# Gyeeta/gyeeta

Hardware: AMD Instinct MI355X
Metric: events/sec ingested + p50/p99 quantile error vs reference, 1→8 MI355X (higher is better)
Workload: dtype int64; 1 GPU; C3/C4: 10000 hosts x 1000 services, raw 24-B tcp_ipv4_resp_event_t stream, uniform over services, 1 window (ingest + window close) per step; service_keys_total=10000000, multi_level_windows=0, td_pend_cap=1920, td_pend_cap_is_library_default=False, exchange=none, exchange_requested=none, exchange_fallback=False

## Files before the change

gyeeta_amd/csrc/gys_kernels.hpp:

```cpp
#pragma once

#include "gys_device.hpp"

namespace gys {

#define GYS_HUGE_VALUE_BITS 20
#define GYS_HUGE_BINS (1u << GYS_HUGE_VALUE_BITS)
#define GYS_ROW_BITS 6
#define GYS_ROW_MASK 0x3Fu
#define GYS_ROW_V6 0x20u
#define GYS_BM_WORDS 32u
#define GYS_STAGED_WORD(tresp, cli_port) ((uint64_t)(((uint32_t)(tresp) << GYS_ROW_BITS) | ((uint32_t)(cli_port) & 0x1Fu)))
#define GYS_STAGED_WORD_FAM(tresp, cli_port, v6) ((uint32_t)(((uint32_t)(tresp) << GYS_ROW_BITS) | ((v6) ? GYS_ROW_V6 : 0u) | ((uint32_t)(cli_port) & 0x1Fu)))

enum { CTR_RESP_EVENTS = 0, CTR_RESP_DROP_RANGE, CTR_RESP_DROP_NOLISTENER, CTR_CONN_EVENTS, CTR_CONN_UNKNOWN, CTR_LSTATE_RECORDS,
       CTR_LSTATE_MISSED, CTR_LSTATE_ERRORS, CTR_LSTATE_DELETED, CTR_TD_MERGES, CTR_TD_MERGE_VALUES, CTR_ACTCONN_RECORDS, CTR_ACTCONN_REMOTE_LISTEN, CTR_ACTCONN_UNKNOWN,
       CTR_CONN_NEW, CTR_CONN_CLOSED, CTR_CONN_CLOSED_NO_NOTIFY, CTR_CONN_CLI_SIDE, CTR_RESP_RUN_OVERFLOW, CTR_NUM };

__global__ void k_table_set(DevTable t, const uint64_t *kv, uint32_t n)
{
	const uint32_t i = blockIdx.x * blockDim.x + threadIdx.x;
	if (i >= n) return;
	const uint64_t key = kv[2u * i];
	uint32_t h = get_uint64_hash(key) & t.mask;
// ... 1219 lines not shown
			const bool fq_on = !SPILL && t0 + 2ull * TILE < e1;
			if (fq_on) {
#pragma unroll
				for (uint32_t j = 0; j < NQ; ++j) fq[j] = ((const uint4 *)p.hll32)[(tile_no & 3u) * ((1u << GYS_HLL_P) / 16u) + j * T + tid];
			}
			for (uint32_t eb0 = 0; eb0 < ntile; eb0 += (uint32_t)FU * T) {
				uint32_t kk[FU], vv[FU];
				uint64_t dd[FU];
#pragma unroll
				for (int j = 0; j < FU; ++j) {
					const uint32_t e = eb0 + (uint32_t)j * T + tid;
					const uint32_t ee = e < ntile ? e : TILE;
					kk[j] = s_key[ee];
					vv[j] = s_val[ee];
				}
				GYS_MEM_FENCE();
#pragma unroll
				for (int j = 0; j < FU; ++j) dd[j] = s_dst[kk[j]];
				GYS_MEM_FENCE();
#pragma unroll
				for (int j = 0; j < FU; ++j) {
					const uint32_t e = eb0 + (uint32_t)j * T + tid;
					if (e < ntile && dd[j]) dstb[dd[j] + e] = vv[j];
				}
			}
			if (fq_on) {
				uint32_t mn = 0xFFFFFFFFu;
#pragma unroll
				for (uint32_t j = 0; j < NQ; ++j) mn = min(min(mn, min(fq[j].x, fq[j].y)), min(fq[j].z, fq[j].w));
				mn = wave_min_u32(mn);
				if (lane == 0) {
					const uint32_t qn = tile_no & 3u;
					atomicMin(&s_fqm[qn], mn);
					atomicMin(&s_floor[tile_no & 1u], min(min(mn, s_fqm[(qn + 1u) & 3u]), min(s_fqm[(qn + 2u) & 3u], s_fqm[(qn + 3u) & 3u])));
				}
			}
		}
		GYS_TICK(11);
	}
#ifdef GYS_RESP_TIMING
	if (!SPILL && lane == 0) {
#pragma unroll
		for (int i = 0; i < 12; ++i) atomicAdd(&g_resp_timing[i], (unsigned long long)tacc[i]);
		atomicAdd(&g_resp_timing[15], 1ull);
	}
#endif
	if (SPILL) return;
	if (DBG && dbg_sink == 0xDEADBEEFu) p.counters[CTR_RESP_EVENTS] = 1;
	if (wmax >= 0) tmax = wmax >> GYS_ROW_BITS;
	tmax = wave_max_i32(tmax);
	if (lane == 0 && tmax != INT32_MIN) atomicMax(&s_gmax, tmax);
	if (ndrop_range) atomicAdd(&s_drop[0], ndrop_range);
	if (ndrop_nol) atomicAdd(&s_drop[1], ndrop_nol);
	__syncthreads();
	if (tid < 64u) {
		unsigned long long cnt = 0, sum = 0;
		if (tid < 15u) {
			for (uint32_t w = 0; w < 16u; ++w) {
				const unsigned long long v = s_gh[w * GYS_GH_STRIDE + tid];
				cnt += v >> 40;
				sum += v & ((1ull << 40) - 1);
			}
			if (cnt) {
				atomicAdd(&p.ghist[2 * tid], cnt);
				atomicAdd(&p.ghist[2 * tid + 1], sum);
			}
		}
		unsigned long long tot = cnt;
#pragma unroll
		for (int d = 8; d >= 1; d >>= 1) tot += (unsigned long long)__shfl_xor((long long)tot, d, 64);
		if (tid == 0 && tot) atomicAdd(&p.ghist[30], tot);
	}
	if (!SHARED) {
		constexpr int KMAX = (int)(2048u / T);
		bool fvalid[KMAX];
		uint32_t fkey[KMAX], fcur[KMAX];
#pragma unroll
		for (int j = 0; j < KMAX; ++j) {
			const uint32_t k = (uint32_t)j * T + tid;
			fvalid[j] = k < L;
			fkey[j] = fvalid[j] ? s_slot[k] : 0u;
			fcur[j] = fvalid[j] ? s_cur[k] : 0u;
		}
		finalize_keys_wg<true, KMAX>(p.fin, &s_fin, tid, lane, fvalid, fkey, fcur);
	}
	if (tid == 0) {
		if (s_gmax != INT32_MIN) atomicMax(p.gmax, (long long)s_gmax);
		if (hd.part == 0u) atomicAdd((unsigned long long *)&p.counters[CTR_RESP_EVENTS], (unsigned long long)(e1 - e0));
		if (s_drop[0]) atomicAdd((unsigned long long *)&p.counters[CTR_RESP_DROP_RANGE], (unsigned long long)s_drop[0]);
		if (s_drop[1]) atomicAdd((unsigned long long *)&p.counters[CTR_RESP_DROP_NOLISTENER], (unsigned long long)s_drop[1]);
	}
}

struct AppendP {
	uint32_t *batch_cnt;
	const uint32_t *off_end;
	const uint32_t *staged;
	uint32_t *td_cur;
	uint32_t *td_pend;
	uint32_t pcap, nsvc;
};

__global__ __launch_bounds__(256) void k_key_append(AppendP p)
{
	const uint32_t lane = threadIdx.x & 63u;
	const uint32_t nchunks = (p.nsvc + 63u) / 64u, nwaves = gridDim.x * 4u;
	for (uint32_t chunk = blockIdx.x * 4u + (threadIdx.x >> 6); chunk < nchunks; chunk += nwaves) {
		const uint32_t key = chunk * 64u + lane;
		const uint32_t m = key < p.nsvc ? p.batch_cnt[key] : 0u;
		unsigned long long todo = __ballot(m != 0);
		if (!todo) continue;
		const uint32_t oend = m ? p.off_end[key] : 0u;
		const uint32_t cur = m ? p.td_cur[key] : 0u;
		if (m) {
			p.batch_cnt[key] = 0;
			p.td_cur[key] = cur + m;
		}
		while (todo) {
			const int k = __ffsll((long long)todo) - 1;
			todo &= todo - 1;
			const uint32_t km = (uint32_t)__shfl((int)m, k, 64), ke = (uint32_t)__shfl((int)oend, k, 64), kc = (uint32_t)__shfl((int)cur, k, 64);
			if ((uint64_t)kc + km > (uint64_t)p.pcap) continue;
			const uint32_t *src = p.staged + (ke - km);
			uint32_t *dst = p.td_pend + (size_t)(chunk * 64u + (uint32_t)k) * p.pcap + kc;
			for (uint32_t i = lane; i < km; i += 64u) dst[i] = src[i];
		}
	}
}

struct DigestP {
	int64_t *td_sum;
	uint32_t *td_cnt;
	TdMeta *td_meta;
	int2 *td_minmax;
	uint32_t *td_pend;
	uint32_t *td_cur;
	uint32_t pcap, nsvc;
	uint32_t pend_cap;
	const uint32_t *staged;
	gys_hist_rec *hist_win, *hist_all;
	uint32_t *bitmap;
};

#define GYS_WAVE_SYNC()                                              \
	do {                                                         \
		__builtin_amdgcn_fence(__ATOMIC_RELEASE, "wavefront"); \
		__builtin_amdgcn_wave_barrier();                     \
		__builtin_amdgcn_fence(__ATOMIC_ACQUIRE, "wavefront"); \
	} while (0)

#define GYS_PACK_ONE (1ull << 40)
#define GYS_PACK_SUM(v) ((v) & (GYS_PACK_ONE - 1))

__device__ __forceinline__ void fold_records(const DigestP &p, uint32_t slot, uint32_t g, bool roll, unsigned long long da, unsigned long long dw,
					     uint32_t n_all, uint32_t n_win, int32_t max_all, int32_t max_win, uint32_t bm, uint32_t bm6)
{
	uint4 *ap = (uint4 *)&p.hist_all[slot] + g, *wp = (uint4 *)&p.hist_win[slot] + g;
	if (n_all) {
		const uint4 a = *ap;
		uint64_t lo = (uint64_t)a.x | ((uint64_t)a.y << 32), hi = (uint64_t)a.z | ((uint64_t)a.w << 32);
		if (g < 15u) {
			lo += da >> 40;
			hi += GYS_PACK_SUM(da);
		} else {
			lo += n_all;
			if ((int64_t)hi < (int64_t)max_all) hi = (uint64_t)(int64_t)max_all;
		}
		if (g == 15u || da) *ap = make_uint4((uint32_t)lo, (uint32_t)(lo >> 32), (uint32_t)hi, (uint32_t)(hi >> 32));
	}
	if (n_win) {
		uint64_t lo = 0, hi = g < 15u ? 0ull : (uint64_t)INT64_MIN;
		if (!roll) {
			const uint4 w = *wp;
			lo = (uint64_t)w.x | ((uint64_t)w.y << 32);
			hi = (uint64_t)w.z | ((uint64_t)w.w << 32);
		}
		if (g < 15u) {
			lo += dw >> 40;
			hi += GYS_PACK_SUM(dw);
		} else {
			lo += n_win;
			if ((int64_t)hi < (int64_t)max_win) hi = (uint64_t)(int64_t)max_win;
		}
		if (roll || g == 15u || dw) *wp = make_uint4((uint32_t)lo, (uint32_t)(lo >> 32), (uint32_t)hi, (uint32_t)(hi >> 32));
		uint32_t *bp = &p.bitmap[(size_t)slot * GYS_BM_WORDS + g];
		const uint32_t old = roll ? 0u : *bp;
		if (roll || (old | bm) != old) *bp = old | bm;
		const uint32_t old6 = bp[16];
		const uint32_t new6 = (roll ? 0u : old6) | bm6;
		if (new6 != old6) bp[16] = new6;
	}
}

struct FoldP {
	DigestP d;
	uint32_t first, n;
	uint32_t *last_tag;
	int64_t *first_sec;
	int64_t tnow;
};

__global__ __launch_bounds__(256) void k_fold(FoldP q)
{
	const DigestP &p = q.d;
	__shared__ unsigned long long s_a_[16][16], s_w_[16][16];
	__shared__ uint32_t s_bm_[16][GYS_BM_WORDS];
	const uint32_t lane = threadIdx.x & 63u, wv = threadIdx.x >> 6;
	const uint32_t row = lane >> 4, g = lane & 15u;
	unsigned long long *s_a = s_a_[wv * 4u + row], *s_w = s_w_[wv * 4u + row];
	uint32_t *s_bm = s_bm_[wv * 4u + row];
	const uint32_t nchunks = (q.n + 63u) / 64u, nwaves = gridDim.x * 4u;
	for (uint32_t chunk = blockIdx.x * 4u + wv; chunk < nchunks; chunk += nwaves) {
		const uint32_t rel = chunk * 64u + lane;
		uint4 mraw = make_uint4(0, 0, 0, 0);
		if (rel < q.n) mraw = *(const uint4 *)&p.td_meta[q.first + rel];
		const unsigned long long todo = __ballot(mraw.x > (mraw.y & 0xFFFFu));
		if (todo) {
			for (uint32_t rd = 0; rd < 16u; ++rd) {
				if (!((todo >> (4u * rd)) & 0xFull)) continue;
				const uint32_t k = rd * 4u + row;
				const uint32_t slot = q.first + chunk * 64u + k;
				uint4 mt;
				mt.x = (uint32_t)__shfl((int)mraw.x, (int)k, 64);
				mt.y = (uint32_t)__shfl((int)mraw.y, (int)k, 64);
				mt.z = (uint32_t)__shfl((int)mraw.z, (int)k, 64);
				mt.w = (uint32_t)__shfl((int)mraw.w, (int)k, 64);
				const uint32_t npend = mt.x, nh = mt.y & 0xFFFFu, nw = mt.y >> 16;
				const uint32_t nwin0 = max(nh, nw);
				const uint32_t m = npend > nh ? npend - nh : 0u;
				s_a[g] = 0;
				s_w[g] = 0;
				s_bm[g] = 0;
				s_bm[g + 16u] = 0;
				GYS_WAVE_SYNC();
				const uint32_t *pend = p.td_pend + (size_t)slot * p.pcap;
				const uint32_t mmax = max(max((uint32_t)__shfl((int)m, 0, 64), (uint32_t)__shfl((int)m, 16, 64)),
							  max((uint32_t)__shfl((int)m, 32, 64), (uint32_t)__shfl((int)m, 48, 64)));
				int32_t lmin = INT32_MAX, lmax = INT32_MIN, wmax = INT32_MIN;
				const uint32_t n_win = npend > nwin0 ? npend - nwin0 : 0u;
				const bool roll = mt.w != mt.z;
				for (uint32_t base = 0; base < mmax; base += 16u) {
					const uint32_t i = nh + base + g;
					if (base + g < m) {
						const uint32_t w = pend[i];
						const int32_t v = (int32_t)(w >> GYS_ROW_BITS);
						const uint32_t b = resp_bucket((int64_t)v);
						const unsigned long long one = GYS_PACK_ONE | (unsigned long long)(uint32_t)v;
						atomicAdd(&s_a[b], one);
						lmin = min(lmin, v);
						lmax = max(lmax, v);
						if (i >= nwin0) {
							atomicAdd(&s_w[b], one);
							const uint32_t r = w & GYS_ROW_MASK;
							atomicOr(&s_bm[r >> 1], (1u << b) << ((r & 1u) * 16u));
							wmax = max(wmax, v);
						}
					}
				}
#pragma unroll
				for (int d = 8; d >= 1; d >>= 1) {
					lmin = min(lmin, __shfl_xor(lmin, d, 64));
					lmax = max(lmax, __shfl_xor(lmax, d, 64));
					wmax = max(wmax, __shfl_xor(wmax, d, 64));
				}
				GYS_WAVE_SYNC();
				if (m) {
					fold_records(p, slot, g, roll, s_a[g], s_w[g], m, n_win, lmax, wmax, s_bm[g], s_bm[g + 16u]);
					if (g == 0) {
						*(uint4 *)&p.td_meta[slot] = make_uint4(npend, npend | (nw << 16), mt.z, n_win ? mt.z : mt.w);
						const int2 mm = p.td_minmax[slot];
						if (lmin < mm.x || lmax > mm.y) p.td_minmax[slot] = make_int2(min(mm.x, lmin), max(mm.y, lmax));
					}
				}
				GYS_WAVE_SYNC();
			}
		}
		if (q.last_tag && rel < q.n) {
			const uint32_t nh = mraw.y & 0xFFFFu, nwin0 = max(nh, mraw.y >> 16);
			q.last_tag[q.first + rel] = mraw.x > nh && mraw.x > nwin0 ? mraw.z : mraw.w;
			if (q.first_sec[q.first + rel] == 0) q.first_sec[q.first + rel] = q.tnow;
		}
	}
}

__device__ __forceinline__ uint32_t td_cluster_of(const uint64_t *T, uint64_t mid2)
{
	uint32_t a = 0, bb = GYS_TD_NB - 1;
	while (a < bb) {
		const uint32_t mid = (a + bb + 1) >> 1;
		if (mid2 >= T[mid]) a = mid; else bb = mid - 1;
	}
	return a;
}

__device__ __forceinline__ uint32_t value_grid(uint32_t v)
{
	if (v < 4u) return v;
	const uint32_t msb = 31u - (uint32_t)__clz((int)v);
	return 4u * (msb - 1u) + ((v >> (msb - 2u)) & 3u);
}
#define GYS_IVL 320u
#define GYS_NBP 256u

__device__ __forceinline__ uint32_t ceil_div_sum_cnt(int64_t cs, uint32_t cc)
{
	uint64_t f = (uint64_t)((double)cs / (double)cc);
	int64_t r = cs - (int64_t)(f * (uint64_t)cc);
	if (r < 0) {
		f--;
		r += cc;
	} else if (r >= (int64_t)cc) {
		f++;
		r -= cc;
	}
	return (uint32_t)(f + (r != 0));
}

struct MergeP {
	DigestP d;
	const MergeEnt *list;
	const uint32_t *count;
	int64_t *out_sum;
	uint32_t *out_cnt;
};

template <uint32_t MAXV, uint32_t NT>
__global__ __launch_bounds__(NT) void k_digest_merge(MergeP q)
{
	const DigestP &p = q.d;
	__shared__ uint32_t s_x[MAXV];
	__shared__ uint32_t s_g[MAXV];
	__shared__ uint32_t s_thr[GYS_NBP];
	__shared__ uint64_t s_cpfx[GYS_NBP + 1];
	__shared__ uint64_t s_T[GYS_NBP];
	__shared__ uint32_t s_imin[GYS_IVL], s_imax[GYS_IVL];
	__shared__ unsigned long long s_osum[GYS_NBP];
	__shared__ uint32_t s_ocnt[GYS_NBP];
	__shared__ uint32_t s_icnt[GYS_IVL];
	__shared__ uint32_t s_ioff[GYS_IVL + 1];
	__shared__ uint32_t s_clt[GYS_IVL];
	__shared__ unsigned long long s_fa[16], s_fw[16];
	__shared__ uint32_t s_fbm[GYS_BM_WORDS];
	__shared__ int32_t s_fmm[3];
	__shared__ uint32_t s_wv[2 * (NT / 64) + 2];
	__shared__ uint64_t s_ww[NT / 64];
	const uint32_t tid = threadIdx.x, lane = tid & 63u, wave = tid >> 6;
	const uint32_t nent = *q.count;
	const bool query = q.out_sum != nullptr;

	for (uint32_t w = blockIdx.x; w < nent; w += gridDim.x) {
		const MergeEnt ent = q.list[w];
		const uint32_t m = ent.nbuf + ent.mrun;
		if (m > MAXV) continue;
		const uint32_t slot = ent.slot;
		const uint4 mt = *(const uint4 *)&p.td_meta[slot];
		const uint32_t nh = query ? ent.nbuf : (mt.y & 0xFFFFu), nw = mt.y >> 16;
		const uint32_t nwin0 = max(nh, nw);
		const uint32_t run0 = ent.off_end - ent.mrun;

		const int64_t *gs = p.td_sum + (size_t)slot * GYS_TD_NB;
		const uint32_t *gc = p.td_cnt + (size_t)slot * GYS_TD_NB;
		uint32_t c0 = 0;
		int64_t sm0 = 0;
		if (tid < GYS_TD_NB) {
			c0 = gc[tid];
			sm0 = gs[tid];
		}
		if (m == 0) {
			if (query && tid < GYS_TD_NB) {
				q.out_sum[(size_t)w * GYS_TD_NB + tid] = sm0;
				q.out_cnt[(size_t)w * GYS_TD_NB + tid] = c0;
			}
			continue;
		}
		uint32_t pos0 = 0, nc = 0;
		uint64_t e0 = 0, nold = 0;
		{
			const unsigned long long b0 = __ballot(c0 != 0);
			const unsigned long long below = lane ? (~0ull >> (64 - lane)) : 0ull;
			const uint64_t inc = wave_incl_scan_u64(c0);
			if (lane == 63u) s_ww[wave] = inc;
			if (lane == 0u) s_wv[wave] = (uint32_t)__popcll(b0);
			__syncthreads();
			uint32_t pbase = 0;
			uint64_t wbase = 0;
#pragma unroll
			for (uint32_t k = 0; k < 4u; ++k) {
				if (k < wave) {
					pbase += s_wv[k];
					wbase += s_ww[k];
				}
				nc += s_wv[k];
				nold += s_ww[k];
			}
			pos0 = pbase + (uint32_t)__popcll(b0 & below);
			e0 = wbase + inc - c0;
		}
		const uint64_t twoN = 2ull * (nold + (uint64_t)m);
		if (tid < GYS_NBP) {
			s_thr[tid] = 0xFFFFFFFFu;
			s_T[tid] = (tid >= 1u && tid < GYS_TD_NB) ? td_threshold(c_td_bnd[tid], twoN) : (tid ? ~0ull : 0ull);
			s_osum[tid] = 0;
			s_ocnt[tid] = 0;
		}
		for (uint32_t i = tid; i < GYS_IVL; i += NT) {
			s_icnt[i] = 0;
			s_imin[i] = 0xFFFFFFFFu;
			s_imax[i] = 0;
			s_clt[i] = 0;
		}
		if (tid < 16u) {
			s_fa[tid] = 0;
			s_fw[tid] = 0;
			s_fbm[tid] = 0;
			s_fbm[tid + 16u] = 0;
		}
		if (tid == 0) {
			s_fmm[0] = INT32_MAX;
			s_fmm[1] = INT32_MIN;
			s_fmm[2] = INT32_MIN;
		}
		__syncthreads();
		if (c0) {
			s_thr[pos0] = ceil_div_sum_cnt(sm0, c0);
			s_cpfx[pos0] = e0;
		}
		if (tid == 0) s_cpfx[nc] = nold;
		__syncthreads();
		{
			const uint32_t *pend = p.td_pend + (size_t)slot * p.pcap;
			int32_t lmin = INT32_MAX, lmax = INT32_MIN, wmax = INT32_MIN;
			for (uint32_t i = tid; i < m; i += NT) {
				const uint32_t word = i < ent.nbuf ? pend[i] : p.staged[run0 + (i - ent.nbuf)];
				const uint32_t uv = word >> GYS_ROW_BITS;
				uint32_t lo = 0;
#pragma unroll
				for (uint32_t step = GYS_NBP / 2; step >= 1u; step >>= 1)
					if (s_thr[lo + step - 1u] <= uv) lo += step;
				const uint32_t iv = lo + value_grid(uv);
				s_x[i] = (iv << 20) | uv;
				atomicAdd(&s_icnt[iv], 1u);
				atomicMin(&s_imin[iv], uv);
				atomicMax(&s_imax[iv], uv);
				atomicAdd(&s_clt[lo + 1], 1u);
				if (i >= nh) {
					const uint32_t b = resp_bucket((int64_t)uv);
					const unsigned long long one = GYS_PACK_ONE | (unsigned long long)uv;
					atomicAdd(&s_fa[b], one);
					lmin = min(lmin, (int32_t)uv);
					lmax = max(lmax, (int32_t)uv);
					if (i >= nwin0) {
						atomicAdd(&s_fw[b], one);
						const uint32_t r = word & GYS_ROW_MASK;
						atomicOr(&s_fbm[r >> 1], (1u << b) << ((r & 1u) * 16u));
						wmax = max(wmax, (int32_t)uv);
					}
				}
			}
			if (!query && m > nh) {
				lmin = wave_min_i32(lmin);
				lmax = wave_max_i32(lmax);
				wmax = wave_max_i32(wmax);
				if (lane == 0) {
					if (lmin != INT32_MAX) atomicMin(&s_fmm[0], lmin);
					if (lmax != INT32_MIN) atomicMax(&s_fmm[1], lmax);
					if (wmax != INT32_MIN) atomicMax(&s_fmm[2], wmax);
				}
			}
		}
		__syncthreads();
		if (wave == 0) {
			uint32_t t[5], gcl[5];
			uint32_t own = 0, gown = 0;
#pragma unroll
			for (int k = 0; k < 5; ++k) {
				t[k] = s_icnt[5u * lane + k];
				gcl[k] = s_clt[5u * lane + k];
				own += t[k];
				gown += gcl[k];
			}
			const uint32_t inc = wave_incl_scan_u32(own), ginc = wave_incl_scan_u32(gown);
			uint32_t ex = inc - own, gex = ginc - gown;
#pragma unroll
			for (int k = 0; k < 5; ++k) {
				s_ioff[5u * lane + k] = ex;
				s_icnt[5u * lane + k] = ex;
				ex += t[k];
				gex += gcl[k];
				s_clt[5u * lane + k] = gex;
			}
			if (lane == 63u) s_ioff[GYS_IVL] = inc;
		}
		__syncthreads();
		for (uint32_t i = tid; i < m; i += NT) {
			const uint32_t x = s_x[i];
			s_g[atomicAdd(&s_icnt[x >> 20], 1u)] = x;
		}
		__syncthreads();
		if (c0) {
			const uint64_t mid2 = 2ull * (e0 + (uint64_t)s_clt[pos0 + 1]) + (uint64_t)c0;
			uint32_t a = 0;
#pragma unroll
			for (uint32_t step = GYS_NBP / 2; step >= 1u; step >>= 1)
				if (mid2 >= s_T[a + step]) a += step;
			atomicAdd(&s_osum[a], (unsigned long long)sm0);
			atomicAdd(&s_ocnt[a], c0);
		}
		for (uint32_t e = tid; e < m; e += NT) {
			const uint32_t x = s_g[e];
			const uint32_t iv = x >> 20;
			uint32_t r = e;
			if (s_imin[iv] != s_imax[iv]) {
				const uint32_t gb = s_ioff[iv], ge = s_ioff[iv + 1];
				r = gb;
				for (uint32_t t = gb; t < ge; ++t) {
					const uint32_t y = s_g[t];
					r += (y < x || (y == x && t < e)) ? 1u : 0u;
				}
			}
			const uint64_t mid2 = 2ull * ((uint64_t)r + s_cpfx[iv - value_grid(x & 0xFFFFFu)]) + 1ull;
			uint32_t a = 0;
#pragma unroll
			for (uint32_t step = GYS_NBP / 2; step >= 1u; step >>= 1)
				if (mid2 >= s_T[a + step]) a += step;
			atomicAdd(&s_osum[a], (unsigned long long)(x & 0xFFFFFu));
			atomicAdd(&s_ocnt[a], 1u);
		}
		__syncthreads();
		if (tid < GYS_TD_NB) {
			int64_t *ws = query ? q.out_sum + (size_t)w * GYS_TD_NB : p.td_sum + (size_t)slot * GYS_TD_NB;
			uint32_t *wc = query ? q.out_cnt + (size_t)w * GYS_TD_NB : p.td_cnt + (size_t)slot * GYS_TD_NB;
			ws[tid] = (int64_t)s_osum[tid];
			wc[tid] = s_ocnt[tid];
		}
		if (!query) {
			const uint32_t n_all = m - nh, n_win = m > nwin0 ? m - nwin0 : 0u;
			if (tid < 16u && n_all) fold_records(p, slot, tid, mt.w != mt.z, s_fa[tid], s_fw[tid], n_all, n_win, s_fmm[1], s_fmm[2], s_fbm[tid], s_fbm[tid + 16u]);
			if (tid == 16u) {
				*(uint4 *)&p.td_meta[slot] = make_uint4(0u, 0u, mt.z, n_win ? mt.z : mt.w);
				p.td_cur[slot] = 0;
				if (n_all) {
					const int2 mm = p.td_minmax[slot];
					if (s_fmm[0] < mm.x || s_fmm[1] > mm.y) p.td_minmax[slot] = make_int2(min(mm.x, s_fmm[0]), max(mm.y, s_fmm[1]));
				}
			}
		}
		__syncthreads();
	}
}

#ifndef GYS_MB_SKIP
#define GYS_MB_SKIP 0
#endif
#define GYS_MB_EXACT 1024u
#define GYS_MB_BINS 2048u
#define GYS_MB_BPT 8u

__device__ __forceinline__ uint32_t mb_bin_clz(uint32_t v)
{
	if (v < GYS_MB_EXACT) return v;
	const uint32_t msb = 31u - (uint32_t)__clz((int)v);
	return GYS_MB_EXACT + (msb - 10u) * 64u + ((v >> (msb - 6u)) & 63u);
}

__device__ __forceinline__ uint32_t mb_bin(uint32_t v)
{
	if (v < GYS_MB_EXACT) return v;
	return (__builtin_bit_cast(uint32_t, (float)v) >> 17) - 7744u;
}

struct MergeBP {
	DigestP d;
	const MergeEnt *list;
	const uint32_t *count;
	int64_t *out_sum;
	uint32_t *out_cnt;
	MergeEnt *slow_list;
	uint32_t *slow_count;
	const double *qs;
	uint32_t nq;
	double *qout;
};

__device__ __forceinline__ double td_quantile_dev(const uint32_t *c_cnt, const unsigned long long *c_sum, const uint32_t *c_wb, uint32_t nc, uint32_t N,
						  int32_t vmin, int32_t vmax, double q)
{
	if (!N) return 0.0;
	if (q < 0.0) q = 0.0;
	if (q > 1.0) q = 1.0;
	const double t = q * (double)N;
	uint32_t lo = 0, hi = nc;
	while (lo < hi) {
		const uint32_t mid = (lo + hi) >> 1;
		if (t < (double)c_wb[mid] + (double)c_cnt[mid] * 0.5) hi = mid; else lo = mid + 1;
	}
	double res;
	if (lo < nc) {
		const double mean = (double)(int64_t)c_sum[lo] / (double)c_cnt[lo];
		const double c = (double)c_wb[lo] + (double)c_cnt[lo] * 0.5;
		if (lo == 0) {
			const double l = (double)vmin;
			res = c <= 0.0 ? mean : l + (mean - l) * (t / c);
		} else {
			const double pm = (double)(int64_t)c_sum[lo - 1] / (double)c_cnt[lo - 1];
			const double pc = (double)c_wb[lo - 1] + (double)c_cnt[lo - 1] * 0.5;
			res = pm + (mean - pm) * ((t - pc) / (c - pc));
		}
	} else {
		const double pm = (double)(int64_t)c_sum[nc - 1] / (double)c_cnt[nc - 1];
		const double pc = (double)c_wb[nc - 1] + (double)c_cnt[nc - 1] * 0.5;
		const double h = (double)vmax, span = (double)N - pc;
		res = span <= 0.0 ? h : pm + (h - pm) * ((t - pc) / span);
	}
	return floor(res + 0.5);
}

#define GYS_MB_BIG_CAP 1024u
#ifndef GYS_MB_WAVES16
#define GYS_MB_WAVES16 5
#endif
template <bool SCAN, uint32_t VPT = 4u>
__global__ __launch_bounds__(256, (VPT == 16u ? GYS_MB_WAVES16 : 8)) void k_digest_bins(MergeBP q_arg)
{
#if defined(__HIP_DEVICE_COMPILE__)
	typedef const MergeBP __attribute__((address_space(4))) *KernargP;
	KernargP q_k = (KernargP)__builtin_amdgcn_kernarg_segment_ptr();
#define GYS_MB_Q_RELOAD() asm volatile("" : "+s"(q_k))
	const MergeBP &q = *(const MergeBP *)q_k;
#else
#define GYS_MB_Q_RELOAD() (void)0
	const MergeBP &q = q_arg;
#endif
	const DigestP &p = q.d;
	static_assert(VPT == 4u || VPT == 8u || VPT == 16u || VPT == 64u, "merges of 1024 / 2048 / 4096 values; 64: up to 16 384, streamed");
	constexpr bool STREAM = VPT > 16u;
	constexpr uint32_t RV = STREAM ? 8u : VPT;
	constexpr bool GROUP = !STREAM;
	constexpr uint32_t GE = GYS_MB_BIG_CAP / 256u;
	__shared__ __align__(16) uint32_t s_bin[GYS_MB_BINS];
	constexpr uint32_t BIG_CAP = GYS_MB_BIG_CAP;
	__shared__ __align__(16) uint32_t s_big[BIG_CAP];
	__shared__ uint32_t s_thr[GYS_NBP];
	__shared__ uint32_t s_cpfx[GYS_NBP + 1];
	__shared__ uint32_t s_T[GYS_NBP];
	__shared__ unsigned long long s_osum[GYS_TD_NB];
	__shared__ uint32_t s_ocnt[GYS_TD_NB];
	__shared__ unsigned long long s_oval[GYS_TD_NB];
	__shared__ unsigned long long s_fa[16], s_fw[16];
	__shared__ uint32_t s_fbm[GYS_BM_WORDS];
	__shared__ int32_t s_fmm[3];
	__shared__ uint32_t s_wv[4], s_ws[4], s_nbig;
	__shared__ uint64_t s_ww[4];
	const uint32_t nent = SCAN ? p.nsvc : *q.count;
	const bool query = SCAN || q.out_sum != nullptr;
	uint32_t bk_first = 0, bk_chg = GYS_MB_BPT;
	if (GYS_MB_BPT * threadIdx.x < GYS_MB_EXACT) {
		bk_first = resp_bucket((int64_t)(GYS_MB_BPT * threadIdx.x));
		for (uint32_t k = GYS_MB_BPT - 1u; k >= 1u; --k)
			if (resp_bucket((int64_t)(GYS_MB_BPT * threadIdx.x + k)) != bk_first) bk_chg = k;
	}

	for (uint32_t w = blockIdx.x; w < nent; w += gridDim.x) {
		uint32_t tid = threadIdx.x;
		GYS_OPAQUE_VGPR(tid);
		GYS_MB_Q_RELOAD();
		const uint32_t lane = tid & 63u, wave = tid >> 6;
		MergeEnt ent;
		if (SCAN) ent = MergeEnt{w, min(p.td_meta[w].npend, p.pend_cap), 0u, 0u};
		else ent = q.list[w];
		const uint32_t m = ent.nbuf + ent.mrun;
		if (m > 256u * VPT) continue;
		const uint32_t slot = ent.slot;
		const uint4 mt = *(const uint4 *)&p.td_meta[slot];
		const uint32_t nh = query ? m : (mt.y & 0xFFFFu), nw = mt.y >> 16;
		const uint32_t nh_mm = SCAN ? (mt.y & 0xFFFFu) : nh;
		const uint32_t nwin0 = max(nh, nw);
		const uint32_t run0 = ent.off_end - ent.mrun;
		uint32_t c0 = 0;
		int64_t sm0 = 0;
		if (tid < GYS_TD_NB) {
			c0 = p.td_cnt[(size_t)slot * GYS_TD_NB + tid];
			sm0 = p.td_sum[(size_t)slot * GYS_TD_NB + tid];
		}
		uint32_t wd[RV];
		const uint32_t *const pend = p.td_pend + (size_t)slot * p.pcap;
		const uint32_t m_s = (uint32_t)__builtin_amdgcn_readfirstlane((int)m), nbuf_s = (uint32_t)__builtin_amdgcn_readfirstlane((int)ent.nbuf);
		const auto load_word = [&](uint32_t base) -> uint32_t {
			const uint32_t i = base + tid;
			if (base + 256u <= nbuf_s) return pend[i];
			uint32_t x = 0;
			if (base < m_s && i < m) x = i < ent.nbuf ? pend[i] : p.staged[run0 + (i - ent.nbuf)];
			return x;
		};
#pragma unroll
		for (uint32_t k = 0; k < RV; ++k) wd[k] = load_word(256u * k);
		if (GYS_MB_SKIP & 32) {
			uint32_t x = c0 ^ (uint32_t)sm0;
#pragma unroll
			for (uint32_t k = 0; k < RV; ++k) x ^= wd[k];
			if (x == 0xDEADBEEFu) p.td_cur[slot] = 1;
			continue;
		}
		if (m == 0 && !SCAN) {
			if (query && tid < GYS_TD_NB) {
				q.out_sum[(size_t)w * GYS_TD_NB + tid] = sm0;
				q.out_cnt[(size_t)w * GYS_TD_NB + tid] = c0;
			}
			continue;
		}
#pragma unroll
		for (uint32_t k = 0; k < GYS_MB_BPT; ++k) s_bin[tid + 256u * k] = 0;
		s_thr[tid] = 0xFFFFFFFFu;
		if (tid < GYS_TD_NB) {
			s_osum[tid] = 0;
			s_ocnt[tid] = 0;
			s_oval[tid] = 0;
		}
		if (tid < 16u) {
			s_fa[tid] = 0;
			s_fw[tid] = 0;
			s_fbm[tid] = 0;
			s_fbm[tid + 16u] = 0;
		}
		if (tid == 0) {
			s_fmm[0] = INT32_MAX;
			s_fmm[1] = INT32_MIN;
			s_fmm[2] = INT32_MIN;
			s_nbig = 0;
		}
		const unsigned long long b0 = __ballot(c0 != 0);
		const uint64_t inc = wave_incl_scan_u64(c0);
		if (lane == 63u) s_ww[wave] = inc;
		if (lane == 0u) s_wv[wave] = (uint32_t)__popcll(b0);
		__syncthreads();
		uint32_t pbase = 0, nc = 0;
		uint64_t wbase = 0, nold64 = 0;
#pragma unroll
		for (uint32_t k = 0; k < 4u; ++k) {
			if (k < wave) {
				pbase += s_wv[k];
				wbase += s_ww[k];
			}
			nc += s_wv[k];
			nold64 += s_ww[k];
		}
		if (nold64 + (uint64_t)m >= (1ull << 31)) {
			if (tid == 0) q.slow_list[atomicAdd(q.slow_count, 1u)] = ent;
			__syncthreads();
			continue;
		}
		if (SCAN && m == 0) {
			if (tid < GYS_TD_NB) {
				s_osum[tid] = (unsigned long long)sm0;
				s_ocnt[tid] = c0;
			}
			__syncthreads();
		} else {
		const uint32_t pos0 = pbase + (uint32_t)__popcll(b0 & (lane ? (~0ull >> (64 - lane)) : 0ull));
		const uint32_t e0 = (uint32_t)(wbase + inc - c0), nold = (uint32_t)nold64;
		const uint32_t twoN = 2u * (nold + m);
		uint32_t thr = 0;
		if (c0) {
			thr = ceil_div_sum_cnt(sm0, c0);
			s_thr[pos0] = thr;
			s_cpfx[pos0] = e0;
			atomicAdd(&s_bin[mb_bin(thr)], 1u << 16);
		}
		if (tid == 0) s_cpfx[nc] = nold;
		s_T[tid] = (tid >= 1u && tid < GYS_TD_NB) ? (uint32_t)td_threshold(c_td_bnd[tid], (uint64_t)twoN) : (tid ? 0xFFFFFFFFu : 0u);
		const bool fold_scan = !query && __builtin_amdgcn_readfirstlane((int)nh) == 0;
		int32_t lmin = INT32_MAX, lmax = INT32_MIN, wmax = INT32_MIN;
		const uint32_t lean_end = min(m_s, (uint32_t)__builtin_amdgcn_readfirstlane((int)nwin0));
		for (uint32_t cb = 0; cb < (STREAM ? m : 1u); cb += 256u * RV) {
		if (STREAM && cb) {
#pragma unroll
			for (uint32_t k = 0; k < RV; ++k) wd[k] = load_word(cb + 256u * k);
		}
#pragma unroll
		for (uint32_t k = 0; k < RV; ++k) {
			const uint32_t base = cb + 256u * k, i = base + tid;
			if (base >= m_s) break;
			if (!SCAN && fold_scan && base + 256u <= lean_end) {
				if (!(GYS_MB_SKIP & 4)) {
					const uint32_t uv = wd[k] >> GYS_ROW_BITS;
					lmin = min(lmin, (int32_t)uv);
					lmax = max(lmax, (int32_t)uv);
					if (uv >= GYS_MB_EXACT) {
						const uint32_t arr = atomicAdd(&s_bin[mb_bin(uv)], 1u) & 0xFFFFu;
						const uint32_t at = atomicAdd(&s_nbig, 1u);
						if (256u * VPT <= BIG_CAP || at < BIG_CAP) s_big[at] = STREAM ? uv : ((arr << 20) | uv);
						atomicAdd(&s_fa[resp_bucket((int64_t)uv)], GYS_PACK_ONE | (unsigned long long)uv);
					} else {
						atomicAdd(&s_bin[uv], 1u);
					}
				}
				continue;
			}
			if (!(i >= m || (GYS_MB_SKIP & 4))) {
			const uint32_t uv = wd[k] >> GYS_ROW_BITS;
			const bool big = uv >= GYS_MB_EXACT;
			if (big) {
				const uint32_t arr = atomicAdd(&s_bin[mb_bin(uv)], 1u) & 0xFFFFu;
				const uint32_t at = atomicAdd(&s_nbig, 1u);
				if (256u * VPT <= BIG_CAP || at < BIG_CAP) s_big[at] = STREAM ? uv : ((arr << 20) | uv);
			} else {
				atomicAdd(&s_bin[uv], 1u);
			}
			if (SCAN && i >= nh_mm) {
				lmin = min(lmin, (int32_t)uv);
				lmax = max(lmax, (int32_t)uv);
			}
			if (i >= nh) {
				lmin = min(lmin, (int32_t)uv);
				lmax = max(lmax, (int32_t)uv);
				const bool win = i >= nwin0;
				if (big || !fold_scan || win) {
					const uint32_t b = resp_bucket((int64_t)uv);
					const unsigned long long one = GYS_PACK_ONE | (unsigned long long)uv;
					if (big || !fold_scan) atomicAdd(&s_fa[b], one);
					if (win) {
						atomicAdd(&s_fw[b], one);
						const uint32_t r = wd[k] & GYS_ROW_MASK;
						atomicOr(&s_fbm[r >> 1], (1u << b) << ((r & 1u) * 16u));
						wmax = max(wmax, (int32_t)uv);
					}
				}
			}
			}
		}
		}
		if ((!query && m > nh) || (SCAN && m > nh_mm)) {
			lmin = wave_min_i32(lmin);
			lmax = wave_max_i32(lmax);
			wmax = wave_max_i32(wmax);
			if (lane == 0) {
				if (lmin != INT32_MAX) atomicMin(&s_fmm[0], lmin);
				if (lmax != INT32_MIN) atomicMax(&s_fmm[1], lmax);
				if (wmax != INT32_MIN) atomicMax(&s_fmm[2], wmax);
			}
		}
		__syncthreads();
		if (256u * VPT > BIG_CAP && s_nbig > BIG_CAP) {
			if (tid == 0) q.slow_list[atomicAdd(q.slow_count, 1u)] = ent;
			__syncthreads();
			continue;
		}
		const uint32_t nbig_s = (uint32_t)__builtin_amdgcn_readfirstlane((int)s_nbig);
		const bool grouped = GROUP && nbig_s != 0u && !(GYS_MB_SKIP & 8);
		uint32_t ge[GE];
#pragma unroll
		for (uint32_t r = 0; r < GE; ++r) ge[r] = 0;
		if (grouped) {
#pragma unroll
			for (uint32_t r = 0; r < GE; ++r)
				if (256u * r < nbig_s && tid + 256u * r < nbig_s) ge[r] = s_big[tid + 256u * r];
		}
		if (!(GYS_MB_SKIP & 8)) {
			uint32_t bv[GYS_MB_BPT], own = 0;
			{
				const uint4 lo4 = ((const uint4 *)s_bin)[2u * tid], hi4 = ((const uint4 *)s_bin)[2u * tid + 1u];
				bv[0] = lo4.x; bv[1] = lo4.y; bv[2] = lo4.z; bv[3] = lo4.w;
				bv[4] = hi4.x; bv[5] = hi4.y; bv[6] = hi4.z; bv[7] = hi4.w;
			}
#pragma unroll
			for (uint32_t k = 0; k < GYS_MB_BPT; ++k) own += bv[k];
			const uint32_t sc = wave_incl_scan_u32(own);
			uint32_t ne_own = 0, ne_sc = 0;
			if (GYS_MB_BPT * 64u * wave < GYS_MB_EXACT) {
#pragma unroll
				for (uint32_t k = 0; k < GYS_MB_BPT; ++k) ne_own += (bv[k] & 0xFFFFu) ? 1u : 0u;
				ne_sc = wave_incl_scan_u32(ne_own);
			}
			if (lane == 63u) {
				s_ws[wave] = sc;
				s_wv[wave] = ne_sc;
			}
			__syncthreads();
			uint32_t run = sc - own;
#pragma unroll
			for (uint32_t k = 0; k < 3u; ++k)
				if (k < wave) run += s_ws[k];
			if (GYS_MB_BPT * 64u * wave < GYS_MB_EXACT && s_nbig <= BIG_CAP / 2u) {
				uint16_t *const s_ne = (uint16_t *)(s_big + BIG_CAP / 2u);
				uint32_t at = ne_sc - ne_own;
#pragma unroll
				for (uint32_t k = 0; k < (GYS_MB_EXACT / (GYS_MB_BPT * 64u)) - 1u; ++k)
					if (k < wave) at += s_wv[k];
#pragma unroll
				for (uint32_t k = 0; k < GYS_MB_BPT; ++k)
					if (bv[k] & 0xFFFFu) s_ne[at++] = (uint16_t)(GYS_MB_BPT * tid + k);
			}
			if (fold_scan && GYS_MB_BPT * tid < GYS_MB_EXACT) {
				uint32_t chg = bk_chg;
				GYS_OPAQUE_VGPR(chg);
				const uint32_t s0 = own & 0xFFFFu;
				uint32_t s1 = 0;
#pragma unroll
				for (uint32_t k = 1; k < GYS_MB_BPT; ++k) s1 += k * (bv[k] & 0xFFFFu);
				uint32_t a0 = s0, a1 = s1;
				if (chg < GYS_MB_BPT) {
					a0 = 0;
					a1 = 0;
#pragma unroll
					for (uint32_t k = 0; k < GYS_MB_BPT - 1u; ++k) {
						const uint32_t c = k < chg ? (bv[k] & 0xFFFFu) : 0u;
						a0 += c;
						a1 += k * c;
					}
				}
				const uint32_t bin0 = GYS_MB_BPT * tid, z0 = s0 - a0;
				const unsigned long long acc0 = ((unsigned long long)(a0 << 8) << 32) | (unsigned long long)(bin0 * a0 + a1);
				const unsigned long long acc1 = ((unsigned long long)(z0 << 8) << 32) | (unsigned long long)(bin0 * z0 + (s1 - a1));
				if (acc0) atomicAdd(&s_fa[bk_first], acc0);
				if (acc1) atomicAdd(&s_fa[bk_first + 1u], acc1);
			}
#pragma unroll
			for (uint32_t k = 0; k < GYS_MB_BPT; ++k) {
				const uint32_t raw = bv[k];
				bv[k] = (run & 0xFFFFu) | (((run >> 16) + (raw >> 16)) << 16);
				run += raw;
			}
			((uint4 *)s_bin)[2u * tid] = make_uint4(bv[0], bv[1], bv[2], bv[3]);
			((uint4 *)s_bin)[2u * tid + 1u] = make_uint4(bv[4], bv[5], bv[6], bv[7]);
		}
		__syncthreads();
		const uint32_t nbig = s_nbig;
		const uint32_t nsmall = s_bin[GYS_MB_EXACT] & 0xFFFFu;
		if (grouped) {
#pragma unroll
			for (uint32_t r = 0; r < GE; ++r)
				if (256u * r < nbig_s && tid + 256u * r < nbig_s) s_big[(s_bin[mb_bin(ge[r] & 0xFFFFFu)] & 0xFFFFu) - nsmall + (ge[r] >> 20)] = ge[r];
			__syncthreads();
		}
		const bool has_old = c0 && !(GYS_MB_SKIP & (2 | 64));
		if (has_old) {
			uint32_t nb = s_bin[mb_bin(thr)] & 0xFFFFu;
			if (thr >= GYS_MB_EXACT) {
				if (GROUP) {
					const uint32_t st = nb - nsmall, cn = (s_bin[mb_bin(thr) + 1u] & 0xFFFFu) - nb;
					for (uint32_t j = 0; j < cn; ++j) nb += (s_big[st + j] & 0xFFFFFu) < thr ? 1u : 0u;
				} else {
				const uint32_t sh = (31u - (uint32_t)__clz((int)thr)) - 6u;
				const uint32_t lo = (thr >> sh) << sh, span = thr - lo;
				const uint32_t n4 = nbig & ~3u;
				for (uint32_t j = 0; j < n4; j += 4u) {
					const uint4 e4 = *(const uint4 *)&s_big[j];
					nb += ((e4.x & 0xFFFFFu) - lo < span ? 1u : 0u) + ((e4.y & 0xFFFFFu) - lo < span ? 1u : 0u) + ((e4.z & 0xFFFFFu) - lo < span ? 1u : 0u) +
					      ((e4.w & 0xFFFFFu) - lo < span ? 1u : 0u);
				}
				for (uint32_t j = n4; j < nbig; ++j) nb += (s_big[j] & 0xFFFFFu) - lo < span ? 1u : 0u;
				}
			}
			const uint32_t mid2 = 2u * (e0 + nb) + c0;
			uint32_t a = 0;
#pragma unroll
			for (uint32_t step = GYS_NBP / 2; step >= 1u; step >>= 1)
				if (mid2 >= s_T[a + step]) a += step;
			atomicAdd(&s_osum[a], (unsigned long long)sm0);
			atomicAdd(&s_ocnt[a], c0);
		}
#ifndef GYS_MB_GROUP
#define GYS_MB_GROUP 1u
#endif
		constexpr uint32_t MBG = SCAN ? 1u : GYS_MB_GROUP;
		const bool compact = MBG == 1u && nbig <= BIG_CAP / 2u;
		if (compact) {
			const uint16_t *const s_ne = (const uint16_t *)(s_big + BIG_CAP / 2u);
			uint32_t n_ne = 0;
			if (!(GYS_MB_SKIP & (1 | 8))) {
#pragma unroll
				for (uint32_t k = 0; k < GYS_MB_EXACT / (GYS_MB_BPT * 64u); ++k) n_ne += s_wv[k];
			}
			for (uint32_t i = tid; i < n_ne; i += 256u) {
				const uint32_t b = s_ne[i];
				const uint32_t bw = s_bin[b];
				uint32_t rem = (s_bin[b + 1u] & 0xFFFFu) - (bw & 0xFFFFu), mid2 = 2u * ((bw & 0xFFFFu) + s_cpfx[bw >> 16]) + 1u, a = 0;
#pragma unroll
				for (uint32_t step = GYS_NBP / 2; step >= 1u; step >>= 1)
					if (mid2 >= s_T[a + step]) a += step;
				while (rem) {
					const uint32_t Tn = s_T[a + 1u];
					const uint32_t kk = min(rem, (Tn - mid2 + 1u) >> 1);
					atomicAdd(&s_oval[a], ((unsigned long long)kk << 40) | (unsigned long long)(kk * b));
					rem -= kk;
					mid2 += 2u * kk;
					++a;
				}
			}
		} else
#pragma unroll
		for (uint32_t k0 = 0; k0 < GYS_MB_EXACT / 256u; k0 += MBG) {
			uint32_t bq[MBG], cq[MBG], mq[MBG], aq[MBG], call = 0;
#pragma unroll
			for (uint32_t u = 0; u < MBG; ++u) {
				bq[u] = tid + 256u * (k0 + u);
				const uint32_t bw = s_bin[bq[u]];
				cq[u] = (GYS_MB_SKIP & 1) ? 0u : (s_bin[bq[u] + 1u] & 0xFFFFu) - (bw & 0xFFFFu);
				mq[u] = 2u * ((bw & 0xFFFFu) + s_cpfx[bw >> 16]) + 1u;
				aq[u] = 0;
				call |= cq[u];
			}
			if (!call) continue;
#pragma unroll
			for (uint32_t step = GYS_NBP / 2; step >= 1u; step >>= 1) {
				uint32_t tq[MBG];
#pragma unroll
				for (uint32_t u = 0; u < MBG; ++u) tq[u] = s_T[aq[u] + step];
#pragma unroll
				for (uint32_t u = 0; u < MBG; ++u)
					if (mq[u] >= tq[u]) aq[u] += step;
			}
#pragma unroll
			for (uint32_t u = 0; u < MBG; ++u) GYS_OPAQUE_VGPR(aq[u]);
#pragma unroll
			for (uint32_t u = 0; u < MBG; ++u) {
				uint32_t rem = cq[u], mid2 = mq[u], a = aq[u];
				const uint32_t b = bq[u];
				while (rem) {
					const uint32_t Tn = s_T[a + 1u];
					const uint32_t kk = min(rem, (Tn - mid2 + 1u) >> 1);
					atomicAdd(&s_oval[a], ((unsigned long long)kk << 40) | (unsigned long long)(kk * b));
					rem -= kk;
					mid2 += 2u * kk;
					++a;
				}
			}
		}
		for (uint32_t j = tid; j < ((GYS_MB_SKIP & (2 | 128)) ? 0u : nbig); j += 256u) {
			uint32_t me;
			if (GROUP) {
				me = ge[0];
#pragma unroll
				for (uint32_t r = 0; r + 1u < GE; ++r) ge[r] = ge[r + 1u];
			} else {
				me = s_big[j];
			}
			const uint32_t uv = me & 0xFFFFFu;
			const uint32_t sh = (31u - (uint32_t)__clz((int)uv)) - 6u;
			uint32_t r = s_bin[mb_bin(uv)] & 0xFFFFu;
			if (GROUP) {
				const uint32_t st = r - nsmall, cn = (s_bin[mb_bin(uv) + 1u] & 0xFFFFu) - r, key = (me << 12) | (me >> 20);
				for (uint32_t jj = 0; jj < cn; ++jj) {
					const uint32_t e = s_big[st + jj];
					r += (((e << 12) | (e >> 20)) < key) ? 1u : 0u;
				}
			} else {
				for (uint32_t jj = 0; jj < nbig; ++jj) {
					const uint32_t e = s_big[jj], u = e & 0xFFFFFu;
					r += ((u >> sh) == (uv >> sh) && (u < uv || (u == uv && jj < j))) ? 1u : 0u;
				}
			}
			uint32_t gap = 0;
#pragma unroll
			for (uint32_t step = GYS_NBP / 2; step >= 1u; step >>= 1)
				if (s_thr[gap + step - 1u] <= uv) gap += step;
			const uint32_t mid2 = 2u * (r + s_cpfx[gap]) + 1u;
			uint32_t a = 0;
#pragma unroll
			for (uint32_t step = GYS_NBP / 2; step >= 1u; step >>= 1)
				if (mid2 >= s_T[a + step]) a += step;
			atomicAdd(&s_oval[a], GYS_PACK_ONE | (unsigned long long)uv);
		}
		__syncthreads();
		if (tid < GYS_TD_NB) {
			const unsigned long long pv = s_oval[tid];
			s_osum[tid] += GYS_PACK_SUM(pv);
			s_ocnt[tid] += (uint32_t)(pv >> 40);
		}
		if (SCAN) __syncthreads();
		}
		if (SCAN) {
			const uint32_t oc = tid < GYS_TD_NB ? s_ocnt[tid] : 0u;
			const unsigned long long os = tid < GYS_TD_NB ? s_osum[tid] : 0ull;
			const unsigned long long ob = __ballot(oc != 0);
			const uint32_t sc = wave_incl_scan_u32(oc);
			if (lane == 63u) s_ws[wave] = sc;
			if (lane == 0u) s_wv[wave] = (uint32_t)__popcll(ob);
			__syncthreads();
			uint32_t pb = 0, wb = 0, ncq = 0, Nq = 0;
#pragma unroll
			for (uint32_t k = 0; k < 4u; ++k) {
				if (k < wave) {
					pb += s_wv[k];
					wb += s_ws[k];
				}
				ncq += s_wv[k];
				Nq += s_ws[k];
			}
			if (oc) {
				const uint32_t pos = pb + (uint32_t)__popcll(ob & (lane ? (~0ull >> (64 - lane)) : 0ull));
				s_thr[pos] = oc;
				s_cpfx[pos] = wb + sc - oc;
				s_osum[pos] = os;
			}
			__syncthreads();
			if (tid < q.nq) {
				const int2 mm = p.td_minmax[slot];
				q.qout[(size_t)slot * q.nq + tid] = td_quantile_dev(s_thr, s_osum, s_cpfx, ncq, Nq, min(mm.x, s_fmm[0]), max(mm.y, s_fmm[1]), q.qs[tid]);
			}
			__syncthreads();
			continue;
		}
		if (GYS_MB_SKIP & 16) {
			if (tid == 208u && !query) {
				*(uint4 *)&p.td_meta[slot] = make_uint4(0u, 0u, mt.z, mt.w);
				p.td_cur[slot] = 0;
			}
			__syncthreads();
			continue;
		}
		if (tid < GYS_TD_NB) {
			int64_t *ws = query ? q.out_sum + (size_t)w * GYS_TD_NB : p.td_sum + (size_t)slot * GYS_TD_NB;
			uint32_t *wc = query ? q.out_cnt + (size_t)w * GYS_TD_NB : p.td_cnt + (size_t)slot * GYS_TD_NB;
			ws[tid] = (int64_t)s_osum[tid];
			wc[tid] = s_ocnt[tid];
		}
		if (!query) {
			const uint32_t n_all = m - nh, n_win = m > nwin0 ? m - nwin0 : 0u;
			if (tid >= 192u && tid < 208u && n_all)
				fold_records(p, slot, tid - 192u, mt.w != mt.z, s_fa[tid - 192u], s_fw[tid - 192u], n_all, n_win, s_fmm[1], s_fmm[2], s_fbm[tid - 192u], s_fbm[tid - 176u]);
			if (tid == 208u) {
				*(uint4 *)&p.td_meta[slot] = make_uint4(0u, 0u, mt.z, n_win ? mt.z : mt.w);
				p.td_cur[slot] = 0;
				if (n_all) {
					const int2 mm = p.td_minmax[slot];
					if (s_fmm[0] < mm.x || s_fmm[1] > mm.y) p.td_minmax[slot] = make_int2(min(mm.x, s_fmm[0]), max(mm.y, s_fmm[1]));
				}
			}
		}
		__syncthreads();
	}
}

struct HugeP {
	DigestP d;
	const MergeEnt *huge_list;
	const uint32_t *huge_count;
	uint32_t *scratch;
};

__global__ __launch_bounds__(256) void k_digest_huge(HugeP p)
{
	__shared__ int64_t s_csum[GYS_TD_NB];
	__shared__ uint32_t s_ccnt[GYS_TD_NB];
	__shared__ uint64_t s_cpfx[GYS_TD_NB + 1];
	__shared__ uint64_t s_T[GYS_TD_NB + 1];
	__shared__ unsigned long long s_osum[GYS_TD_NB];
	__shared__ unsigned long long s_ocnt[GYS_TD_NB];
	__shared__ uint32_t s_part[256];
	__shared__ uint32_t s_wave[4];
	__shared__ unsigned long long s_ha[32], s_hw[32];
	__shared__ uint32_t s_bm[GYS_BM_WORDS];
	__shared__ uint32_t s_nc;
	__shared__ int32_t s_min, s_max, s_wmax;
	uint32_t *bins = p.scratch + (size_t)blockIdx.x * GYS_HUGE_BINS;
	const uint32_t nh_list = *p.huge_count;
	const uint32_t BPT = GYS_HUGE_BINS / 256u;

	for (uint32_t w = blockIdx.x; w < nh_list; w += gridDim.x) {
		const MergeEnt ent = p.huge_list[w];
		const uint32_t slot = ent.slot;
		const uint32_t m = ent.mrun, npend = ent.nbuf;
		const uint32_t start = ent.off_end - m;
		const uint4 mt = *(const uint4 *)&p.d.td_meta[slot];
		const uint32_t nh = mt.y & 0xFFFFu, nw = mt.y >> 16;
		const uint32_t nwin0 = max(nh, nw);
		const uint32_t *pend = p.d.td_pend + (size_t)slot * p.d.pcap;
		for (uint32_t i = threadIdx.x; i < GYS_HUGE_BINS / 4u; i += 256u) ((uint4 *)bins)[i] = make_uint4(0, 0, 0, 0);
		if (threadIdx.x < GYS_TD_NB) {
			s_osum[threadIdx.x] = 0;
			s_ocnt[threadIdx.x] = 0;
		}
		if (threadIdx.x < 32u) {
			s_ha[threadIdx.x] = 0;
			s_hw[threadIdx.x] = 0;
		}
		if (threadIdx.x >= 160u && threadIdx.x < 160u + GYS_BM_WORDS) s_bm[threadIdx.x - 160u] = 0;
		if (threadIdx.x == 0) {
			const int64_t *gs = p.d.td_sum + (size_t)slot * GYS_TD_NB;
			const uint32_t *gc = p.d.td_cnt + (size_t)slot * GYS_TD_NB;
			uint32_t nc = 0;
			uint64_t run = 0;
			for (uint32_t j = 0; j < GYS_TD_NB; ++j) {
				if (gc[j]) {
					s_csum[nc] = gs[j];
					s_ccnt[nc] = gc[j];
					s_cpfx[nc] = run;
					run += gc[j];
					nc++;
				}
			}
			s_cpfx[nc] = run;
			s_nc = nc;
			s_min = INT32_MAX;
			s_max = INT32_MIN;
			s_wmax = INT32_MIN;
		}
		__syncthreads();
		const uint32_t nc = s_nc;
		const uint64_t nold = s_cpfx[nc];
		const uint64_t twoN = 2ull * (nold + (uint64_t)m + (uint64_t)npend);
		if (threadIdx.x >= 1 && threadIdx.x < GYS_TD_NB) s_T[threadIdx.x] = td_threshold(c_td_bnd[threadIdx.x], twoN);
		if (threadIdx.x == 0) s_T[GYS_TD_NB] = ~0ull;
		{
			int32_t lmin = INT32_MAX, lmax = INT32_MIN, wmax = INT32_MIN;
			for (uint32_t i = threadIdx.x; i < npend + m; i += 256u) {
				const uint32_t word = i < npend ? pend[i] : p.d.staged[start + (i - npend)];
				const uint32_t v = (word >> GYS_ROW_BITS) & (GYS_HUGE_BINS - 1u);
				atomicAdd(&bins[v], 1u);
				if (i >= nh) {
					const uint32_t hb = resp_bucket((int64_t)v);
					atomicAdd(&s_ha[2 * hb], 1ull);
					atomicAdd(&s_ha[2 * hb + 1], (unsigned long long)v);
					lmin = min(lmin, (int32_t)v);
					lmax = max(lmax, (int32_t)v);
					if (i >= nwin0) {
						atomicAdd(&s_hw[2 * hb], 1ull);
						atomicAdd(&s_hw[2 * hb + 1], (unsigned long long)v);
						const uint32_t row = word & GYS_ROW_MASK;
						const uint32_t bit = (1u << hb) << ((row & 1u) * 16u);
						if ((s_bm[row >> 1] & bit) == 0) atomicOr(&s_bm[row >> 1], bit);
						wmax = max(wmax, (int32_t)v);
					}
				}
			}
			atomicMin(&s_min, lmin);
			atomicMax(&s_max, lmax);
			atomicMax(&s_wmax, wmax);
		}
		__syncthreads();
		__builtin_amdgcn_fence(__ATOMIC_ACQUIRE, "agent");
		uint32_t part = 0;
		{
			const uint4 *b4 = (const uint4 *)(bins + threadIdx.x * BPT);
			for (uint32_t i = 0; i < BPT / 4u; ++i) {
				const uint4 v = b4[i];
				part += v.x + v.y + v.z + v.w;
			}
		}
		uint32_t tot;
		const uint32_t pfx = block_exclusive_scan_256(part, s_wave, &tot);
		s_part[threadIdx.x] = pfx;
		__syncthreads();
		if (threadIdx.x < nc) {
			const int64_t cs = s_csum[threadIdx.x];
			const uint32_t cc = s_ccnt[threadIdx.x];
			uint64_t lt = 0;
			if (cs > 0) {
				int64_t vmax = (cs - 1) / (int64_t)cc;
				if (vmax >= (int64_t)GYS_HUGE_BINS) vmax = GYS_HUGE_BINS - 1;
				const uint32_t owner = (uint32_t)vmax / BPT;
				lt = s_part[owner];
				for (uint32_t b = owner * BPT; b <= (uint32_t)vmax; ++b) lt += bins[b];
			}
			const uint64_t mid2 = 2ull * (s_cpfx[threadIdx.x] + lt) + (uint64_t)cc;
			const uint32_t cl = td_cluster_of(s_T, mid2);
			atomicAdd(&s_osum[cl], (unsigned long long)cs);
			atomicAdd(&s_ocnt[cl], (unsigned long long)cc);
		}
		{
			uint64_t r0 = pfx;
			uint32_t ci = 0;
			const uint32_t vbeg = threadIdx.x * BPT;
			{
				uint32_t lo = 0, hi = nc;
				const int64_t v = (int64_t)vbeg;
				while (lo < hi) {
					const uint32_t mid = (lo + hi) >> 1;
					if (s_csum[mid] <= v * (int64_t)s_ccnt[mid]) lo = mid + 1; else hi = mid;
				}
				ci = lo;
			}
			for (uint32_t b = vbeg; b < vbeg + BPT; ++b) {
				const uint32_t c = bins[b];
				if (!c) continue;
				const int64_t v = (int64_t)b;
				while (ci < nc && s_csum[ci] <= v * (int64_t)s_ccnt[ci]) ci++;
				const uint64_t le = s_cpfx[ci];
				const uint64_t first = 2ull * (r0 + le) + 1ull, last = first + 2ull * (uint64_t)(c - 1u);
				uint32_t cl = td_cluster_of(s_T, first);
				const uint32_t cl_last = td_cluster_of(s_T, last);
				uint64_t rbeg = r0;
				for (; cl <= cl_last; ++cl) {
					uint64_t rend;
					if (cl == cl_last) {
						rend = r0 + c;
					} else {
						const uint64_t Tn = s_T[cl + 1];
						rend = (Tn / 2ull) - le;
						if (rend > r0 + c) rend = r0 + c;
					}
					if (rend > rbeg) {
						const uint64_t k = rend - rbeg;
						atomicAdd(&s_osum[cl], (unsigned long long)(k * (uint64_t)v));
						atomicAdd(&s_ocnt[cl], (unsigned long long)k);
						rbeg = rend;
					}
				}
				r0 += c;
			}
		}
		__syncthreads();
		if (threadIdx.x < GYS_TD_NB) {
			p.d.td_sum[(size_t)slot * GYS_TD_NB + threadIdx.x] = (int64_t)s_osum[threadIdx.x];
			p.d.td_cnt[(size_t)slot * GYS_TD_NB + threadIdx.x] = (uint32_t)s_ocnt[threadIdx.x];
		}
		{
			const uint32_t n_all = npend + m - nh, n_win = npend + m - nwin0;
			const uint32_t t = threadIdx.x - 128u;
			if (threadIdx.x >= 128u && t < 16u) {
				gys_hist_serial *ap = (gys_hist_serial *)&p.d.hist_all[slot] + t, *wp = (gys_hist_serial *)&p.d.hist_win[slot] + t;
				const bool roll = mt.w != mt.z;
				gys_hist_serial av = *ap;
				if (t < 15u) {
					av.count += s_ha[2 * t];
					av.sum += (int64_t)s_ha[2 * t + 1];
				} else {
					av.count += n_all;
					if (av.sum < (int64_t)s_max) av.sum = (int64_t)s_max;
				}
				*ap = av;
				if (n_win) {
					gys_hist_serial wv;
					if (roll) {
						wv.count = 0;
						wv.sum = t < 15u ? 0 : INT64_MIN;
					} else {
						wv = *wp;
					}
					if (t < 15u) {
						wv.count += s_hw[2 * t];
// ... 1720 lines not shown
```

Before: 76.93 billion events/s.

## Use fp32 reciprocal fast path for ceil-div and rebalance per-thread work assignment

Replaces the double-precision division in ceil_div_sum_cnt with an fp32 reciprocal estimate plus integer correction, falling back to the f64 path for large quotients or uncorrected cases. It also reverses the thread-to-big-entry mapping (255-tid) and rotates thread assignment for the non-empty bin loop after the first pass. The intent is to cut the cost of slow f64 division and to spread tail work across waves, so the waves finishing the small-bin loop are not the same ones that take big-entry work. The remapping must stay consistent between the loads and the later use of ge[], and the fp32 path adds branches.

```diff
diff --git a/gyeeta_amd/csrc/gys_kernels.hpp b/gyeeta_amd/csrc/gys_kernels.hpp
--- a/gyeeta_amd/csrc/gys_kernels.hpp
+++ b/gyeeta_amd/csrc/gys_kernels.hpp
@@ -1545,7 +1545,7 @@
 #define GYS_IVL 320u
 #define GYS_NBP 256u
 
-__device__ __forceinline__ uint32_t ceil_div_sum_cnt(int64_t cs, uint32_t cc)
+__device__ __forceinline__ uint32_t ceil_div_sum_cnt_f64(int64_t cs, uint32_t cc)
 {
 	uint64_t f = (uint64_t)((double)cs / (double)cc);
 	int64_t r = cs - (int64_t)(f * (uint64_t)cc);
@@ -1557,6 +1557,32 @@
 		r -= cc;
 	}
 	return (uint32_t)(f + (r != 0));
+}
+
+__device__ __forceinline__ uint32_t ceil_div_sum_cnt(int64_t cs, uint32_t cc)
+{
+#if defined(__HIP_DEVICE_COMPILE__)
+	const float rc = __builtin_amdgcn_rcpf((float)cc);
+#else
+	const float rc = 1.0f / (float)cc;
+#endif
+	const float fq = __builtin_fmaf((float)(uint32_t)((uint64_t)cs >> 32), 4294967296.0f, (float)(uint32_t)cs) * rc;
+	if (fq < 4194304.0f) {
+		uint32_t f = (uint32_t)fq;
+		int64_t r = cs - (int64_t)((uint64_t)f * (uint64_t)cc);
+		for (int k = 0; k < 2; ++k) {
+			if (r < 0) {
+				f--;
+				r += cc;
+			}
+			if (r >= (int64_t)cc) {
+				f++;
+				r -= cc;
+			}
+		}
+		if (r >= 0 && r < (int64_t)cc) return f + (r != 0);
+	}
+	return ceil_div_sum_cnt_f64(cs, cc);
 }
 
 struct MergeP {
@@ -2090,13 +2116,14 @@
 		}
 		const uint32_t nbig_s = (uint32_t)__builtin_amdgcn_readfirstlane((int)s_nbig);
 		const bool grouped = GROUP && nbig_s != 0u && !(GYS_MB_SKIP & 8);
+		const uint32_t big0 = 255u - tid;
 		uint32_t ge[GE];
 #pragma unroll
 		for (uint32_t r = 0; r < GE; ++r) ge[r] = 0;
 		if (grouped) {
 #pragma unroll
 			for (uint32_t r = 0; r < GE; ++r)
-				if (256u * r < nbig_s && tid + 256u * r < nbig_s) ge[r] = s_big[tid + 256u * r];
+				if (256u * r < nbig_s && big0 + 256u * r < nbig_s) ge[r] = s_big[big0 + 256u * r];
 		}
 		if (!(GYS_MB_SKIP & 8)) {
 			uint32_t bv[GYS_MB_BPT], own = 0;
@@ -2172,7 +2199,7 @@
 		if (grouped) {
 #pragma unroll
 			for (uint32_t r = 0; r < GE; ++r)
-				if (256u * r < nbig_s && tid + 256u * r < nbig_s) s_big[(s_bin[mb_bin(ge[r] & 0xFFFFFu)] & 0xFFFFu) - nsmall + (ge[r] >> 20)] = ge[r];
+				if (256u * r < nbig_s && big0 + 256u * r < nbig_s) s_big[(s_bin[mb_bin(ge[r] & 0xFFFFFu)] & 0xFFFFu) - nsmall + (ge[r] >> 20)] = ge[r];
 			__syncthreads();
 		}
 		const bool has_old = c0 && !(GYS_MB_SKIP & (2 | 64));
@@ -2214,7 +2241,10 @@
 #pragma unroll
 				for (uint32_t k = 0; k < GYS_MB_EXACT / (GYS_MB_BPT * 64u); ++k) n_ne += s_wv[k];
 			}
-			for (uint32_t i = tid; i < n_ne; i += 256u) {
+			const uint32_t n_ne_s = (uint32_t)__builtin_amdgcn_readfirstlane((int)n_ne);
+			for (uint32_t i0 = 0; i0 < n_ne_s; i0 += 256u) {
+				const uint32_t i = i0 + (i0 ? ((tid - 64u) & 255u) : tid);
+				if (i >= n_ne_s) continue;
 				const uint32_t b = s_ne[i];
 				const uint32_t bw = s_bin[b];
 				uint32_t rem = (s_bin[b + 1u] & 0xFFFFu) - (bw & 0xFFFFu), mid2 = 2u * ((bw & 0xFFFFu) + s_cpfx[bw >> 16]) + 1u, a = 0;
@@ -2269,7 +2299,7 @@
 				}
 			}
 		}
-		for (uint32_t j = tid; j < ((GYS_MB_SKIP & (2 | 128)) ? 0u : nbig); j += 256u) {
+		for (uint32_t j = big0; j < ((GYS_MB_SKIP & (2 | 128)) ? 0u : nbig); j += 256u) {
 			uint32_t me;
 			if (GROUP) {
 				me = ge[0];
```

Measured after the change: 77.06 billion events/s (median of 3 runs). About the same (+0.2%).
